# yakir1991/LoRa-SDR-Lightweight-Standalone-Library-

Hardware: AMD Instinct MI355X
Metric: Msymbols/s dechirp+FFT+argmax @ SF7 & SF12, 1/2/4/8 GPU; % HBM roofline (higher is better)
Workload: dtype f32; 1 GPU; SF7 BW125 osr1 LEGACY lora_demodulate + fused dechirp, 15625 frames x (2 sync + 64 data) symbols per GPU, noiseless; launch=eager, streams=3, sf=7, osr=1, frames_per_gpu=15625, data_symbols_per_frame=64, parallelism=frames sharded x1, no collective (gloo timing only), symbols_ok=True

## Files before the change

### lora-sdr-lightweight-standalone-library-_amd/csrc/lora_demod_fast.hip

```cpp
#include "../../include/lora_mi355x.h"
#include "lora_internal.h"

#include <algorithm>
#include <cstdlib>
#include <type_traits>
#include <utility>

#pragma clang fp contract(off)

namespace lora {
namespace {


template <int SF>
struct Geo {
  static constexpr int N = 1 << SF;
  static constexpr bool SMALL = SF <= 5;
  static constexpr int P = SMALL ? N : 16;
  static constexpr int T = N / P;
  static constexpr int R1 = SMALL ? N : ((SF & 1) ? 8 : 16);
  static constexpr int LOGR1 = SMALL ? SF : ((SF & 1) ? 3 : 4);
  static constexpr int G1 = P / R1;
  static constexpr bool R2FIRST = (SF & 1) != 0;
  static constexpr int X = N / R1;
// ... 676 lines not shown
      const auto xb = __builtin_amdgcn_permlane16_swap(best, best, false, false);
      const auto xs = __builtin_amdgcn_permlane16_swap(sec, sec, false, false);
      const auto xp = __builtin_amdgcn_permlane16_swap(pm, pm, false, false);
      best = xb[0], sec = xs[0], pm = xp[0];
      top2_merge(best, sec, pm, xb[1], xs[1], xp[1]);
    } else {
      static_assert(O == 32, "wave64");
      const auto xb = __builtin_amdgcn_permlane32_swap(best, best, false, false);
      const auto xs = __builtin_amdgcn_permlane32_swap(sec, sec, false, false);
      const auto xp = __builtin_amdgcn_permlane32_swap(pm, pm, false, false);
      best = xb[0], sec = xs[0], pm = xp[0];
      top2_merge(best, sec, pm, xb[1], xs[1], xp[1]);
    }
    spec_reduce_step<2 * O, W>(best, sec, pm);
  }
}
template <int SF>
__device__ __forceinline__ void spec_reduce(uint32_t& best, uint32_t& sec, float& pmf, int tid, uint32_t* scratch) {
  constexpr int T = Geo<SF>::T;
  uint32_t pm = __float_as_uint(pmf);
  spec_reduce_step<1, (T < 64 ? T : 64)>(best, sec, pm);
  if constexpr (T > 64) {
    const int w = tid >> 6;
    if ((tid & 63) == 0) {
      scratch[3 * w] = best;
      scratch[3 * w + 1] = sec;
      scratch[3 * w + 2] = pm;
    }
    __syncthreads();
    constexpr int WPS = T / 64;
    const int wb = (w / WPS) * WPS;
    best = scratch[3 * wb];
    sec = scratch[3 * wb + 1];
    pm = scratch[3 * wb + 2];
#pragma unroll
    for (int q = 1; q < WPS; ++q)
      top2_merge(best, sec, pm, scratch[3 * (wb + q)], scratch[3 * (wb + q) + 1], scratch[3 * (wb + q) + 2]);
  }
  pmf = __uint_as_float(pm);
}

template <int SF>
constexpr int demod_waves_per_eu() {
  return SF >= 6 ? 4 : 1;
}

template <int SF, bool SPEC>
constexpr int demod_twl_entries() {
  if constexpr (!SPEC || SF < 6) {
    return 0;
  } else {
    using G = Geo<SF>;
    return (G::RA == 16 ? 15 : 3) * G::MA_A;
  }
}


template <int SF>
constexpr size_t spec_dtl_offset() {
  return (((size_t)Geo<SF>::SPW * lds_row<SF>() + demod_twl_entries<SF, true>()) * sizeof(cf) + 15) & ~(size_t)15;
}
template <int SF>
constexpr bool spec_dtab() {
  return Geo<SF>::WAVE_LOCAL && Geo<SF>::NPASS == 2 &&
         4 * (spec_dtl_offset<SF>() + 2 * sizeof(cf) * Geo<SF>::N) <= 160 * 1024;
}
template <int SF>
constexpr size_t spec_lds_bytes() {
  constexpr bool pf2 = Geo<SF>::WAVE_LOCAL && Geo<SF>::NPASS == 2;
  return pf2 ? spec_dtl_offset<SF>() + (spec_dtab<SF>() ? 2 * sizeof(cf) * Geo<SF>::N : 16 * 8 * Geo<SF>::T)
             : sizeof(cf) * ((size_t)Geo<SF>::SPW * lds_row<SF>() + demod_twl_entries<SF, true>());
}

#define LORA_SPEC_BLOCKS(SPB, dblocks, frames, sync) ((dblocks) + ((sync) ? (2 * (frames) + (SPB) - 1) / (SPB) : 0))
template <int SF>
struct SpecGrid {
  static constexpr int SPB = Geo<SF>::WAVE_LOCAL ? 64 / Geo<SF>::T : Geo<SF>::SPW;
  static constexpr int BPG = Geo<SF>::WAVE_LOCAL ? 4 : 1;
  __host__ __device__ static constexpr int bpf(int per) { return (per + SPB - 1) / SPB; }
  static constexpr int64_t groups(int64_t frames, int per, bool sync) {
    return (LORA_SPEC_BLOCKS(SPB, frames * bpf(per), frames, sync) + BPG - 1) / BPG;
  }
};

__device__ __forceinline__ __amdgpu_buffer_rsrc_t raw_rsrc(const void* p) {
  return __builtin_amdgcn_make_buffer_rsrc(const_cast<void*>(p), (short)0, 0x7fffffff, 0x00020000);
}

struct SpecBlk {
  int64_t f, base;
  int s, jl, d, cg;
  bool valid, mis, nbr;
  float rate;
  int toff;
};
template <int SF, int SPM, int DW, bool RECIP>
__device__ __forceinline__ void spec_decode(const KArgs& a, int64_t bb, int bpf, int per, int gi, int l, bool fdiv,
                                            uint64_t mq, SpecBlk& B) {
  constexpr int SPB = SpecGrid<SF>::SPB, S0 = SPM == 2 ? 0 : 2;
  const __attribute__((address_space(4))) FrameParams* fps =
      (const __attribute__((address_space(4))) FrameParams*)a.fp_spec;
  if constexpr (RECIP)
    B.f = fdiv ? (bpf == 1 ? bb : (int64_t)(((uint64_t)(uint32_t)bb * mq) >> 32)) : bb / bpf;
  else
    B.f = bb / bpf;
  B.jl = (int)(bb - B.f * bpf) * SPB + gi;
  B.valid = B.jl < per;
  B.s = S0 + (B.valid ? B.jl : per - 1);
  B.rate = SPM == 2 ? 0.0f : fps[B.f].rate;
  B.toff = SPM == 2 ? 0 : fps[B.f].t_off;
  sym_base(B.s, Geo<SF>::N, a.frame_len, B.toff, B.base, B.cg);
  if constexpr (SPM == 1) B.cg = 0;
  B.d = (int)(B.base & (DW - 1));
  B.mis = __builtin_amdgcn_readfirstlane(__ballot(Geo<SF>::NPASS == 3 ? l < B.d : B.d != 0) != 0);
  B.nbr = false;
}
template <int SF>
__device__ __forceinline__ bool spec_next_is_neighbour(const KArgs& a, const SpecBlk& B, int per, int gi) {
  int64_t bnext;
  int cgn;
  sym_base(B.s + 1, Geo<SF>::N, a.frame_len, B.toff, bnext, cgn);
  return gi < SpecGrid<SF>::SPB - 1 && B.jl + 1 < per && bnext == B.base + Geo<SF>::N;
}

template <int SF, bool DTAB, bool DTL>
__device__ __forceinline__ float4 spec_table_pair(int pp, __amdgpu_buffer_rsrc_t rd, int vt, bool cg0, const cf* dq,
                                                  const float4* dl) {
  constexpr int N = Geo<SF>::N, T = Geo<SF>::T;
  if constexpr (DTAB) {
    const cf d0 = dq[2 * pp * T], d1 = dq[(2 * pp + 1) * T];
    return float4{d0.re, d0.im, d1.re, d1.im};
  } else if constexpr (DTL) {
    return cg0 ? dl[pp * T]
               : __builtin_bit_cast(float4, __builtin_amdgcn_raw_buffer_load_b128(rd, vt, pp * (N + T) * 16, 0));
  } else {
    return __builtin_bit_cast(float4, __builtin_amdgcn_raw_buffer_load_b128(rd, vt, pp * (N + T) * 16, 0));
  }
}
template <int SF, bool DTAB, bool DTL, int NP>
__device__ __forceinline__ void spec_table(const KArgs& a, int cg, int lr, const cf* dtab, const float4* dtl,
                                           float4 (&dt)[NP]) {
  const __amdgpu_buffer_rsrc_t rd = raw_rsrc(a.downP);
  const int vt = (cg + lr) * 16;
  bool cg0 = false;
  if constexpr (DTL && !DTAB) cg0 = __builtin_amdgcn_readfirstlane(__ballot(cg != 0) == 0);
#pragma unroll
  for (int pp = 0; pp < NP; ++pp) dt[pp] = spec_table_pair<SF, DTAB, DTL>(pp, rd, vt, cg0, dtab + cg + lr, dtl + lr);
}
template <int MODE, bool MAX, int P>
__device__ __forceinline__ float spec_dechirp_max(const v2f (&ld)[P + 1], const float4* dt, cf (&in)[P]) {
#pragma unroll
  for (int q = 0; q < P; ++q) in[q] = cf{ld[q].x, ld[q].y};
  if constexpr (MODE == 0) {
#pragma unroll
    for (int pp = 0; pp < P / 2; ++pp) {
      in[2 * pp] = pk_cmul_ref(in[2 * pp], cf{dt[pp].x, dt[pp].y});
      in[2 * pp + 1] = pk_cmul_ref(in[2 * pp + 1], cf{dt[pp].z, dt[pp].w});
    }
  }
  float pm = 0.0f;
  if constexpr (MAX) {
#pragma unroll
    for (int q = 0; q < P; ++q) pm = amax3(pm, in[q]);
  }
  return pm;
}
// ... 53 lines not shown
  const float scale = (legacy && p.scaled) ? p.scale : 1.0f;

  constexpr bool FMA = SPEC && FAST;
  constexpr int NTW = demod_twl_entries<SF, SPEC>();
  static_assert(NTW <= 256, "one staged twiddle per thread");
  cf* twl = rows + (size_t)SPW * rowc;
  cf tv{0.0f, 0.0f};
  if constexpr (NTW > 0) {
    if (tid < NTW) tv = a.twTA ? a.twTA[tid] : a.tw[twT_index(N, G::MA_A, tid / G::MA_A, tid % G::MA_A)];
  }
  cf in[P], z[P];
  if (SPEC && MODE == 0 && a.downP)
    gather_points<SF, true>(a, x, l, 1, N, cg, 1, true, 1.0f, in);
  else
    gather_points<SF>(a, x, l, osr, step, cg, legacy ? 1 : 2, dech, SPEC ? 1.0f : scale, in);
  if constexpr (NTW > 0) {
    if (tid < NTW) twl[tid] = tv;
    if constexpr (G::WAVE_LOCAL) __syncthreads();
  }
  float pm = 0.0f;
  if constexpr (SPEC) {
#pragma unroll
    for (int q = 0; q < P; ++q) pm = amax3(pm, in[q]);
  }
  rotate_place<SF, !RAW, FAST, FMA>(in, z, start, p.rate, hann, a.win, l);
  if constexpr (SPEC) asm volatile("" : "+v"(pm));
  float sec = 0.0f;
  const uint64_t lkey =
      fft_key<SF, false, FMA, (NTW > 0)>(z, rows + (size_t)g * rowc, l, a, SPEC ? &sec : nullptr, twl);
  const uint64_t key = symbol_key<SF>(lkey, tid, red);
  if (l == 0 && valid && a.syms) a.syms[f * a.sym_stride + (s - s0)] = (uint16_t)key_index(key);
  if constexpr (SPEC) {
    float r2 = lkey == key ? sec : key_value(lkey);
    group_reduce2<SF>(r2, pm, tid, reinterpret_cast<float*>(smem + 64));
    if (l == 0 && valid) {
      const int64_t per = a.total - s0;
      reinterpret_cast<float2*>(a.spec_marg)[f * per + (s - s0)] = make_float2(sqrtf(key_value(key)) - sqrtf(r2), pm);
    }
  }
}


template <int SF, int MODE, bool HANN = false, int OSRV = 1, int SPM = 0>
__global__ void __launch_bounds__(256) __attribute__((amdgpu_waves_per_eu(demod_waves_per_eu<SF>())))
k_spec_demod(KArgs a, int64_t frames, int rowc, int64_t gstride) {
  using G = Geo<SF>;
  constexpr int N = G::N, T = G::T, P = G::P, SPW = G::SPW;
  constexpr bool WL = G::WAVE_LOCAL;
  using SG = SpecGrid<SF>;
  constexpr int SPB = SG::SPB;
  constexpr int BPG = SG::BPG;
  constexpr int NTW = demod_twl_entries<SF, true>();
  constexpr bool OSRN = OSRV != 1;
  constexpr bool FOLD = SF <= 8 && !HANN;
  static_assert(P == 16 && (MODE == 0 || MODE == 1), "SF >= 6, LEGACY (osr 1, or OSRN)");
  static_assert(OSRV == 0 || OSRV == 1 || OSRV == 2 || OSRV == 4, "osr 1, 2, 4 or run time");
  static_assert(NTW <= 256, "one staged twiddle per thread");
  extern __shared__ __attribute__((aligned(16))) unsigned char smem[];
  __shared__ uint32_t red3[3 * 4];
  cf* rows = reinterpret_cast<cf*>(smem);
  cf* twl = rows + (size_t)SPW * rowc;
  const int tot = a.total;
  constexpr bool API = SPM == 1, RAWM = SPM == 2;
  constexpr int S0 = RAWM ? 0 : 2;
  const int per = tot - S0;
  constexpr bool DTL = WL && G::NPASS == 2 && !OSRN && MODE == 0;
  constexpr bool DTAB = DTL && spec_dtab<SF>();
  float4* dtl = reinterpret_cast<float4*>(smem + spec_dtl_offset<SF>());
  cf* dtab = reinterpret_cast<cf*>(smem + spec_dtl_offset<SF>());
  if (SPM != 0 && blockIdx.x == 0 && threadIdx.x < kFixStripes) a.fix_count[16 * threadIdx.x] = 0;
  if constexpr (NTW > 0) {
    const int tid = threadIdx.x;
    if (tid < NTW) twl[tid] = a.twTA ? a.twTA[tid] : a.tw[twT_index(N, G::MA_A, tid / G::MA_A, tid % G::MA_A)];
    if constexpr (DTAB) {
      for (int i = tid; i < 2 * N; i += 256) dtab[i] = a.down[i];
    } else if constexpr (DTL) {
      static_assert(8 * T <= 256, "one staged pair per thread");
      if (tid < 8 * T) dtl[tid] = reinterpret_cast<const float4*>(a.downP)[(tid / T) * (N + T) + tid % T];
    }
    __syncthreads();
  }
  const int bpf = SG::bpf(per);
  const int64_t dblocks = frames * bpf;
  const int64_t blocks = LORA_SPEC_BLOCKS(SPB, dblocks, frames, SPM == 0);
  const int64_t groups = (blocks + BPG - 1) / BPG;
  const int wave = __builtin_amdgcn_readfirstlane((int)(threadIdx.x >> 6));

  auto run_block = [&](auto sync_c, int64_t b, int64_t fb, int rb) {
    constexpr bool SYNC = decltype(sync_c)::value;
    int tid = threadIdx.x;
    asm volatile("" : "+v"(tid));
    const int g = SPW == 1 ? 0 : tid / T;
    const int l = tid % T;
    const int gi = WL ? (g % SPB) : g;
    int64_t f, fu;
    int s;
    bool valid;
    int rel = 0;
    if constexpr (!SYNC) {
      f = fu = fb;
      const int jl = rb * SPB + gi;
      valid = jl < per;
      s = S0 + (valid ? jl : per - 1);
    } else {
      const int64_t k0 = (b - dblocks) * SPB;
      int64_t k = k0 + gi;
      valid = k < 2 * frames;
      if (!valid) k = 2 * frames - 1;
      f = k >> 1;
      s = (int)(k & 1);
      fu = k0 >> 1;
      rel = (int)((f - fu) * a.frame_stride * 8);
    }
    const FrameParams fp = RAWM ? FrameParams{} : a.fp_spec[f];
    const float rate = RAWM ? 0.0f : fp.rate;
    const int toff = RAWM ? 0 : fp.t_off;
    const int step = OSRN ? a.step : N;
    int64_t base;
    int cg;
    sym_base(s, step, a.frame_len, toff, base, cg);
    if constexpr (API) cg = 0;
    cf in[P];
    float pm = 0.0f;
    int lr = l;
    if constexpr (OSRN) {
      const int osr = OSRV ? OSRV : a.osr;
      const __amdgpu_buffer_rsrc_t rx = raw_rsrc(a.iq + fu * a.frame_stride);
      const __amdgpu_buffer_rsrc_t rd = raw_rsrc(a.down);
      const int vo = rel + (int)(base + (int64_t)l * osr) * 8;
      const int vt = (cg + l * osr) * 8;
      const int so = T * osr * 8;
      if constexpr (OSRV == 4) {
        const bool odd = (l & 1) != 0;
        lr = odd ? T / 2 + (l >> 1) : (l >> 1);
        const int vo2 = rel + (int)base * 8 + 16 * l;
        const int vt2 = (cg + 2 * l) * 8;
#pragma unroll
        for (int q = 0; q < P; ++q) {
          cf e0;
#pragma unroll
          for (int h = 0; h < 2; ++h) {
            const int i = 2 * q + h;
            const float4 y2 = __builtin_bit_cast(float4, __builtin_amdgcn_raw_buffer_load_b128(rx, vo2, i * 2 * T * 8, 2 ));
            cf y0 = cf{y2.x, y2.y}, y1 = cf{y2.z, y2.w};
            if constexpr (MODE == 0) {
              const float4 d2 = __builtin_bit_cast(float4, __builtin_amdgcn_raw_buffer_load_b128(rd, vt2, i * 2 * T * 8, 0));
              y0 = pk_cmul_ref(y0, cf{d2.x, d2.y});
              y1 = pk_cmul_ref(y1, cf{d2.z, d2.w});
            }
            if constexpr (!SYNC) pm = amax3(amax3(pm, y0), y1);
            if (h == 0) {
              e0 = y0;
            } else {
              const cf m = cf{__int_as_float(__builtin_amdgcn_update_dpp(0, __float_as_int(y0.re), 0x111, 0xF, 0xF, false)),
                              __int_as_float(__builtin_amdgcn_update_dpp(0, __float_as_int(y0.im), 0x111, 0xF, 0xF, false))};
              in[q] = odd ? m : e0;
            }
          }
        }
      } else if constexpr (OSRV == 2) {
#pragma unroll
        for (int q = 0; q < P; ++q) {
          const float4 y2 = __builtin_bit_cast(float4, __builtin_amdgcn_raw_buffer_load_b128(rx, vo, q * so, 2 ));
          cf y0 = cf{y2.x, y2.y}, y1 = cf{y2.z, y2.w};
          if constexpr (MODE == 0) {
            const float4 d2 = __builtin_bit_cast(float4, __builtin_amdgcn_raw_buffer_load_b128(rd, vt, q * so, 0));
            y0 = pk_cmul_ref(y0, cf{d2.x, d2.y});
            y1 = pk_cmul_ref(y1, cf{d2.z, d2.w});
          }
          if constexpr (!SYNC) pm = amax3(amax3(pm, y0), y1);
          in[q] = y0;
        }
      } else {
#pragma unroll
      for (int q = 0; q < P; ++q) {
        for (int k = 0; k < osr; ++k) {
          cf y = __builtin_bit_cast(cf, __builtin_amdgcn_raw_buffer_load_b64(rx, vo + 8 * k, q * so, 2 ));
          if constexpr (MODE == 0)
            y = pk_cmul_ref(y, __builtin_bit_cast(cf, __builtin_amdgcn_raw_buffer_load_b64(rd, vt + 8 * k, q * so, 0)));
          if constexpr (!SYNC) pm = amax3(pm, y);
          if (k == 0) in[q] = y;
        }
      }
      }
    } else {
    constexpr int D = T < 8 ? T : 8;
    const int d = (int)(base & (D - 1));
    lr = (l - d) & (T - 1);
    v2f ld[P + 1];
    const __amdgpu_buffer_rsrc_t rx = raw_rsrc(a.iq + fu * a.frame_stride);
    const int vo = rel + (int)(base - d + l) * 8;
    float4 dt[MODE == 0 ? P / 2 : 1];
    const __amdgpu_buffer_rsrc_t rd = raw_rsrc(a.downP);
    const int vt = (cg + lr) * 16;
    constexpr int AUX = SYNC ? 0 : 2;
#pragma unroll
    for (int pp = 0; pp < P / 2; ++pp) {
      if constexpr (MODE == 0) dt[pp] = spec_table_pair<SF, false, false>(pp, rd, vt, false, nullptr, nullptr);
#pragma unroll
      for (int q = 2 * pp; q < 2 * pp + 2; ++q)
        ld[q] = __builtin_bit_cast(v2f, __builtin_amdgcn_raw_buffer_load_b64(rx, vo, q * T * 8, AUX));
    }
    if (__builtin_amdgcn_readfirstlane(__ballot(l < d) != 0)) {
      const bool late = l < d;
      ld[P] = __builtin_bit_cast(
          v2f, __builtin_amdgcn_raw_buffer_load_b64(rx, late ? vo : vo - T * 8, P * T * 8, AUX));
#pragma unroll
      for (int q = 0; q < P; ++q) ld[q] = late ? ld[q + 1] : ld[q];
    }
    pm = spec_dechirp_max<MODE, !SYNC>(ld, dt, in);
    }
    cf z[P], wz[P];
    {
      v2f F[P];
      spec_factors<SF>(rate, lr, F);
      spec_rotate_place<SF, HANN, FOLD>(in, z, F, a.win, lr, wz);
    }
    asm volatile("" : "+v"(pm));
    const uint64_t lk = fft_key<SF, false, true, (NTW > 0), true, false, NoHook, FOLD>(
        z, rows + (size_t)g * rowc, lr, a, nullptr, twl, nullptr, NoHook{}, nullptr, wz);
    const uint32_t lbest = (uint32_t)lk;
    uint32_t best = lbest, sec = (uint32_t)(lk >> 32);
    spec_reduce<SF>(best, sec, pm, tid, red3);
    if (valid) {
      constexpr int NG = (G::NPASS == 2 ? P / G::RA : P / G::RB);
      constexpr int ML = G::NPASS == 2 ? G::MA_A : G::MA_B;
      const int o = (int)(best & 15u);
      const uint32_t idx = (uint32_t)(lr + T * (o % NG) + ML * (o / NG));
      const float margin = spec_margin(best, sec);
      uint2* mg = reinterpret_cast<uint2*>(a.spec_marg) + f * tot + s;
      if constexpr (!SYNC) {
        if (lbest == best && a.syms) a.syms[f * a.sym_stride + (s - S0)] = (uint16_t)idx;
        if (l == 0) *mg = make_uint2(__float_as_uint(margin), __float_as_uint(pm));
      } else {
        if (lbest == best) *mg = make_uint2(__float_as_uint(margin), idx);
      }
    }
    block_sync<WL>();
  };
  int64_t grp0 = blockIdx.x;
  constexpr bool PL = SF == 7 && !HANN && WL && G::NPASS == 2 && !OSRN;
  const int64_t bstep = gstride * BPG;
  if constexpr (PL) {
    static_assert(T == 8 && P == 16 && G::G1 == 2 && G::R1 == 8 && G::LOGR1 == 3 && FOLD, "SF7 geometry");
    static_assert(MODE != 0 || (DTAB && NTW > 0), "the fused dechirp reads the staged doubled table");
    constexpr int DL = 16;
    const int tid0 = threadIdx.x;
    const int g = tid0 / T;
    const int l = tid0 % T;
    const int gi = g % SPB;
    float4 nx[P / 2 + 1];
    const bool fdiv = (uint64_t)dblocks * (uint64_t)bpf < (1ull << 32);
    const uint64_t mq = ((1ull << 32) + (uint64_t)bpf - 1) / (uint64_t)bpf;
    auto issue = [&](int64_t bb, SpecBlk& B) {
      spec_decode<SF, SPM, DL, true>(a, bb, bpf, per, gi, l, fdiv, mq, B);
      const __amdgpu_buffer_rsrc_t rx = raw_rsrc(a.iq + B.f * a.frame_stride);
      const int vo = (int)(B.base - B.d) * 8 + 16 * l;
#pragma unroll
      for (int j = 0; j < P / 2; ++j)
        nx[j] = __builtin_bit_cast(float4, __builtin_amdgcn_raw_buffer_load_b128(rx, vo, j * DL * 8, 2 ));
      if (B.mis) {
        B.nbr = spec_next_is_neighbour<SF>(a, B, per, gi);
        if (!B.nbr) {
          if (2 * l < B.d) {
            const v2f e0 = __builtin_bit_cast(v2f, __builtin_amdgcn_raw_buffer_load_b64(rx, vo, (P / 2) * DL * 8, 2));
            nx[P / 2].x = e0.x;
            nx[P / 2].y = e0.y;
          }
          if (2 * l + 1 < B.d) {
            const v2f e1 = __builtin_bit_cast(v2f, __builtin_amdgcn_raw_buffer_load_b64(rx, vo + 8, (P / 2) * DL * 8, 2));
            nx[P / 2].z = e1.x;
            nx[P / 2].w = e1.y;
          }
        }
      }
    };
    int64_t b = grp0 * BPG + wave;
    SpecBlk nb{};
    if (b < dblocks) issue(b, nb);
    for (; b < dblocks; b += bstep, grp0 += gstride) {
      const SpecBlk B = nb;
      float4(&ld)[P / 2 + 1] = nx;
      const int d = B.d;
      int r[2];
      bool late[2];
#pragma unroll
      for (int h = 0; h < 2; ++h) {
        const int x = 2 * l + h - d;
        late[h] = x < 0;
        r[h] = x & (DL - 1);
      }
      cf dv[MODE == 0 ? P : 1];
      if constexpr (MODE == 0) {
#pragma unroll
        for (int h = 0; h < 2; ++h) {
          const cf* dq = dtab + B.cg + r[h];
#pragma unroll
          for (int m = 0; m < P / 2; ++m) dv[h + 2 * m] = dq[DL * m];
        }
      }
      cf in[P];
      if (B.mis) {
        const int src = ((int)__lane_id() + T) & 63;
        const float4 n0 = {__shfl(ld[0].x, src, 64), __shfl(ld[0].y, src, 64), __shfl(ld[0].z, src, 64),
                           __shfl(ld[0].w, src, 64)};
        if (B.nbr) ld[P / 2] = n0;
#pragma unroll
        for (int m = 0; m < P / 2; ++m) {
          in[2 * m] = late[0] ? cf{ld[m + 1].x, ld[m + 1].y} : cf{ld[m].x, ld[m].y};
          in[2 * m + 1] = late[1] ? cf{ld[m + 1].z, ld[m + 1].w} : cf{ld[m].z, ld[m].w};
        }
      } else {
#pragma unroll
        for (int m = 0; m < P / 2; ++m) {
          in[2 * m] = cf{ld[m].x, ld[m].y};
          in[2 * m + 1] = cf{ld[m].z, ld[m].w};
        }
      }
      constexpr bool EARLY = MODE == 0;
      if constexpr (EARLY) {
        __builtin_amdgcn_sched_barrier(0);
        if (b + bstep < dblocks) issue(b + bstep, nb);
        __builtin_amdgcn_sched_barrier(0);
      }
      if constexpr (MODE == 0) {
#pragma unroll
        for (int q = 0; q < P; ++q) in[q] = pk_cmul_ref(in[q], dv[q]);
      }
// ... 45 lines not shown
      const int vo = (int)(B.base - B.d + l) * 8;
#pragma unroll
      for (int q = 0; q < P; ++q)
        nx[q] = __builtin_bit_cast(v2f, __builtin_amdgcn_raw_buffer_load_b64(rx, vo, q * T * 8, 2 ));
      if (B.mis) {
        if constexpr (P3) {
          nx[P] = __builtin_bit_cast(
              v2f, __builtin_amdgcn_raw_buffer_load_b64(rx, l < B.d ? vo : vo - T * 8, P * T * 8, 2 ));
        } else {
          B.nbr = spec_next_is_neighbour<SF>(a, B, per, gi);
          if (l < B.d && !B.nbr)
            nx[P] = __builtin_bit_cast(v2f, __builtin_amdgcn_raw_buffer_load_b64(rx, vo, P * T * 8, 2 ));
        }
      }
    };
    int64_t b = grp0 * BPG + (WL ? wave : 0);
    SpecBlk nb{};
    if (b < dblocks) issue(b, nb);
    for (; b < dblocks; b += bstep, grp0 += gstride) {
      const SpecBlk B = nb;
      v2f(&ld)[P + 1] = nx;
      const int d = B.d;
      const int lr = (l - d) & (T - 1);
      float4 dt[MODE == 0 ? P / 2 : 1];
      if constexpr (MODE == 0) spec_table<SF, DTAB, DTL>(a, B.cg, lr, dtab, dtl, dt);
      if (B.mis) {
        const bool late = l < d;
        if constexpr (!P3) {
          const int src = ((int)__lane_id() + T) & 63;
          const v2f n0 = {__shfl(ld[0].x, src, 64), __shfl(ld[0].y, src, 64)};
          if (late && B.nbr) ld[P] = n0;
        }
#pragma unroll
        for (int q = 0; q < P; ++q) ld[q] = late ? ld[q + 1] : ld[q];
      }
      cf in[P];
      float pm = spec_dechirp_max<MODE, true>(ld, dt, in);
      constexpr int NTB = G::RB == 16 ? 15 : 3;
      cf wb[P3 ? (P / G::RB) * NTB : 1];
      if constexpr (P3) {
#pragma unroll
        for (int gg = 0; gg < P / G::RB; ++gg) load_tw2<G::RB, G::MA_B>(wb + gg * NTB, (lr + T * gg) % G::MA_B, a.twTB2);
      }
      asm volatile("" : "+v"(pm));
      cf z[P], wz[P];
      {
        v2f F[P];
        spec_factors<SF>(B.rate, lr, F);
        spec_rotate_place<SF, HANN, FOLD>(in, z, F, a.win, lr, wz);
      }
      asm volatile("" : "+v"(pm));
      auto prefetch = [&]() {
        if (b + bstep < dblocks) issue(b + bstep, nb);
      };
      int cpre[G::G1];
      uint64_t lk;
      if constexpr (P3) {
#pragma unroll
        for (int h = 0; h < G::G1; ++h) cpre[h] = d == 0 ? cown[h] : (int)(a.rev[lr + T * h] >> G::LOGR1);
        lk = fft_key<SF, false, true, (NTW > 0), true, true, decltype(prefetch), FOLD>(
            z, rows + (size_t)g * rowc, lr, a, nullptr, twl, cpre, prefetch, wb, wz);
      } else {
        __builtin_amdgcn_sched_barrier(0);
        prefetch();
        __builtin_amdgcn_sched_barrier(0);
#pragma unroll
        for (int h = 0; h < G::G1; ++h) cpre[h] = __shfl(cown[h], lane0 + lr, 64);
        lk = fft_key<SF, false, true, (NTW > 0), true, true, NoHook, FOLD>(
            z, rows + (size_t)g * rowc, lr, a, nullptr, twl, cpre, NoHook{}, nullptr, wz);
      }
      const uint32_t lbest = (uint32_t)lk;
      uint32_t best = lbest, sec = (uint32_t)(lk >> 32);
      spec_reduce<SF>(best, sec, pm, tid0, red3);
      if (B.valid) spec_store_symbol<SF, S0>(a, B.f, B.s, l, lr, lbest, best, sec, pm);
      block_sync<WL>();
    }
  }
  for (int64_t grp = grp0; grp < groups; grp += gstride) {
    const int64_t b = grp * BPG + (WL ? wave : 0);
    if (WL && b >= blocks) break;
    if (b < dblocks) {
      const int64_t fb = b / bpf;
      run_block(std::false_type{}, b, fb, (int)(b - fb * bpf));
    } else {
      run_block(std::true_type{}, b, 0, 0);
    }
  }
}

template <int SF>
struct EstGeo {
  static constexpr int T = Geo<SF>::T;
  static constexpr int BLOCK = T >= 64 ? 256 : 64;
  static constexpr int SPB = BLOCK / T;
  static constexpr bool PAIR = SF >= 7 && Geo<SF>::WAVE_LOCAL && Geo<SF>::NPASS == 2;
};

template <int SF, int MODE>
__device__ __forceinline__ uint32_t exact_symbol(const KArgs& a, const cf* __restrict__ x,
                                                           const FrameParams& q, int s, cf* row, int l, int tid,
                                                           uint64_t* red) {
  using G = Geo<SF>;
  constexpr int N = G::N, P = G::P;
  constexpr bool DYN = MODE == 2;
  const int step = DYN ? a.step : N;
  const int osr = DYN ? a.osr : 1;
  const bool legacy = DYN ? a.mode != LORA_MODE_API : true;
  const bool dech = DYN ? (legacy && a.dechirp) : (MODE == 0);
  const bool hann = a.hann != 0;
  int64_t base;
  int cg;
  sym_base(s, step, a.frame_len, q.t_off, base, cg);
  const float start = q.rate * ((float)((uint32_t)s * (uint32_t)N) + (float)q.t_off / (float)osr);
  cf in[P], z[P];
  gather_points<SF>(a, x + base, l, osr, step, cg, legacy ? 1 : 2, dech, (legacy && q.scaled) ? q.scale : 1.0f, in);
  rotate_place<SF, true>(in, z, start, q.rate, hann, a.win, l);
  uint64_t key = fft_key<SF, false>(z, row, l, a);
  key = symbol_key<SF>(key, tid, red);
  block_sync<G::WAVE_LOCAL>();
  return key_index(key);
}

constexpr double kHwSinCosErr = 2.0e-7;

template <int SF, int LANES>
__device__ __forceinline__ void certify_list(const KArgs& a, int64_t f, const FrameParams& q, bool valid, int li) {
  constexpr int N = 1 << SF;
  const FrameParams qs = a.fp_spec[f];
  const int per = a.total - 2;
  const bool same_t = qs.t_off == q.t_off;
  constexpr int T = N >= 16 ? N / 16 : 1;
  const double u = 1.0 / 16777216.0;
  const double E = (8.0 * SF + 42.0) * u;
  const double drate = fabs((double)q.rate - (double)qs.rate);
  const double rmax = fmax(fabs((double)q.rate), fabs((double)qs.rate));
  const double tabs = (double)abs(q.t_off);
  const double e_spec = 36.0 * u * rmax * T + 16.0 * (1.87e-7 + 1.4143 * kHwSinCosErr) + 2.6e-6 + 9.6e-7;
  auto certified = [&](double d, double wmax, int s) {
    const double n1 = 2.0 * N * wmax;
    const double L = (double)(s + 1) * N + tabs;
    const double e_ref = u * rmax * (L + 2.0 * N);
    const double B = n1 * (drate * N + e_ref + e_spec + 2.0 * E);
    return same_t && d > 4.0 * B + 0x1p-60;
  };
  const uint2* __restrict__ mg = reinterpret_cast<const uint2*>(a.spec_marg) + f * a.total;
  bool sync_rej = false;
  if (a.mode != LORA_MODE_API) {
    const uint2 e = mg[li < 2 ? li : 0];
    const bool ok = certified((double)__uint_as_float(e.x), (double)__uint_as_float(a.maxbits[f]), li & 1);
    const uint32_t ok1 = (uint32_t)__shfl_down((int)ok, 1, 64), i1 = (uint32_t)__shfl_down((int)e.y, 1, 64);
    if (li == 0 && valid) {
      if (ok && ok1) {
        if (a.sync) {
          const unsigned shift = a.sf > 4 ? a.sf - 4 : 0;
          a.sync[f] = (uint8_t)((((e.y >> shift) & 0x0f) << 4) | ((i1 >> shift) & 0x0f));
        }
      } else {
        sync_rej = true;
      }
    }
  }
  if (valid) {
    uint64_t rejbits = 0;
#pragma unroll 8
    for (int j = li, k = 0; j < per; j += LANES, ++k) {
      const uint2 v = mg[2 + j];
      if (!certified((double)__uint_as_float(v.x), (double)__uint_as_float(v.y), 2 + j)) rejbits |= 1ull << k;
// ... 352 lines not shown

template <int SF, int MODE>
__global__ void __launch_bounds__(256) __attribute__((amdgpu_waves_per_eu(2)))
k_spec_fix(KArgs a, int rowc, int64_t grid) {
  using G = Geo<SF>;
  constexpr int T = G::T, SPW = G::SPW;
  extern __shared__ __attribute__((aligned(16))) unsigned char smem[];
  __shared__ uint64_t red[4];
  const int tid = threadIdx.x;
  const int g = SPW == 1 ? 0 : tid / T;
  const int l = tid % T;
  int64_t count = 0;
  unsigned cnt[kFixStripes];
#pragma unroll
  for (int t = 0; t < kFixStripes; ++t) {
    cnt[t] = __builtin_nontemporal_load(a.fix_count + 16 * t);
    count += cnt[t];
  }
  if (blockIdx.x == 0 && tid == 0 && count > 0) atomicAdd(a.spec_fix, (unsigned)count);
  cf* row = reinterpret_cast<cf*>(smem) + (size_t)g * rowc;
  for (int64_t r0 = 0; (int64_t)blockIdx.x + grid * r0 < count; r0 += SPW) {
    const int64_t i = (int64_t)blockIdx.x + grid * (r0 + g);
    const bool valid = i < count;
    int64_t k = valid ? i : count - 1;
    int t = 0;
#pragma unroll
    for (int u = 0; u < kFixStripes - 1; ++u)
      if (t == u && k >= (int64_t)cnt[u]) {
        k -= cnt[u];
        ++t;
      }
    const uint32_t* list = a.fix_list + 2 * (size_t)t * (size_t)a.fix_cap;
    const int64_t f = list[2 * k];
    const uint32_t j = list[2 * k + 1];
    const bool sync = j == 0xFFFFFFFFu;
    const FrameParams q = a.fp[f];
    const cf* __restrict__ x = a.iq + f * a.frame_stride;
    int lo = l;
    asm volatile("" : "+v"(lo));
    const int js = (a.mode == LORA_MODE_RAW ? 0 : 2) + (int)j;
    const uint32_t i0 = exact_symbol<SF, MODE>(a, x, q, sync ? 0 : js, row, lo, tid, red);
    const bool any_sync = G::WAVE_LOCAL ? __any(sync) : __syncthreads_or(sync);
    uint32_t i1 = 0;
    if (any_sync) i1 = exact_symbol<SF, MODE>(a, x, q, sync ? 1 : js, row, lo, tid, red);
    if (l == 0 && valid) {
      if (!sync) {
        if (a.syms) a.syms[f * a.sym_stride + j] = (uint16_t)i0;
      } else if (a.sync) {
        const unsigned shift = a.sf > 4 ? a.sf - 4 : 0;
        a.sync[f] = (uint8_t)((((i0 >> shift) & 0x0f) << 4) | ((i1 >> shift) & 0x0f));
      }
    }
  }
}

template <int SF>
int row_complex() {
  return lds_row<SF>();
}

template <int SF, int MODE>
__global__ void __launch_bounds__(64) __attribute__((amdgpu_waves_per_eu(4)))
k_est_split(KArgs a, int64_t frames, int rowc) {
  using G = Geo<SF>;
  constexpr int N = G::N, T = G::T, P = G::P;
  constexpr int FPW = 64 / (2 * T);
  static_assert(2 * T <= 64 && P == 16, "SF 6-9");
  constexpr bool dech = MODE == 0;
  extern __shared__ __attribute__((aligned(16))) unsigned char smem[];
  __shared__ FrameParams sp[FPW];
  __shared__ float tail[FPW][2][4];
  const int tid = threadIdx.x;
  if (blockIdx.x == 0 && tid < kFixStripes) a.fix_count[16 * tid] = 0;
  const int g2 = tid / T;
  const int fg = g2 >> 1;
  const int sym = g2 & 1;
  const int l = tid % T;
  const int l2 = tid % (2 * T);
  const int64_t f0 = (int64_t)blockIdx.x * FPW + fg;
  const bool valid = f0 < frames;
  const int64_t f = valid ? f0 : frames - 1;
  const cf* __restrict__ x = a.iq + f * a.frame_stride;
  cf* row = reinterpret_cast<cf*>(smem) + (size_t)g2 * rowc;
  auto frame_max = [&](float v) {
#pragma unroll
    for (int o = T; o > 0; o >>= 1) v = fmaxf(v, __shfl_xor(v, o, 64));
    return v;
  };
  FrameParams q;
  {
    cf in[P], z[P];
    gather_points<SF>(a, x + (int64_t)sym * N, l, 1, N, 0, 1, dech, 1.0f, in);
    float mo = 0.0f;
#pragma unroll
    for (int k = 0; k < P; ++k) mo = amax3(mo, in[k]);
    asm volatile("" : "+v"(mo));
    const float m01 = frame_max(mo);
    const int scaled = m01 > 1.0f;
    const float scale = scaled ? 1.0f / m01 : 1.0f;
    if (scaled) {
#pragma unroll
      for (int k = 0; k < P; ++k) in[k] = cscale(in[k], scale);
    }
    rotate_place<SF, false>(in, z, 0.0f, 0.0f, a.hann != 0, a.win, l);
    uint64_t key = fft_key<SF, true>(z, row, l, a);
    key = group_max(key, T);
    if (l == 0) {
      const uint32_t idx = key_index(key);
      const uint32_t im1 = idx > 0 ? idx - 1 : N - 1, ip1 = idx < (uint32_t)N - 1 ? idx + 1 : 0;
      const cf L = row[lds_slot<SF>((int)im1)], R = row[lds_slot<SF>((int)ip1)], B = row[lds_slot<SF>((int)idx)];
      const float fi = detect_findex(key_value(key), L, R);
      const bool take = key_value(key) > 0.0f;
      tail[fg][sym][0] = take ? (float)idx : 0.0f;
      tail[fg][sym][1] = take ? fi : 0.0f;
      tail[fg][sym][2] = lm_atan2f(take ? B.im : 0.0f, take ? B.re : 0.0f);
    }
    wave_sync();
    if (l2 == 0) {
      float sum_index = 0.0f, phase_diff = 0.0f;
      sum_index += tail[fg][0][0] + tail[fg][0][1];
      sum_index += tail[fg][1][0] + tail[fg][1][1];
      float d = tail[fg][1][2] - tail[fg][0][2];
      while (d > PI_F) d -= 2.0f * PI_F;
      while (d < -PI_F) d += 2.0f * PI_F;
      phase_diff += d;
      const float avg_index = sum_index / 2.0f;
      const float cfo_coarse = avg_index / (float)N;
      const float cfo_fine = (phase_diff / 1.0f) / (2.0f * PI_F * (float)N);
      const float cfo = cfo_coarse + cfo_fine;
      const float frac = avg_index - floorf(avg_index + 0.5f);
      const float avg_t = (float)0u / 2.0f;
      const float toff = avg_t - frac * (float)N * 1.0f;
      FrameParams qe;
      qe.cfo = cfo;
      qe.toff = toff;
      qe.t_off = (int)roundf(toff);
      qe.rate = -2.0f * PI_F * cfo / (float)N;
      qe.scale = scale;
      qe.scaled = scaled;
      qe.pad0 = qe.pad1 = 0;
      sp[fg] = qe;
      if (valid) a.fp_spec[f] = qe;
    }
    wave_sync();
    q = sp[fg];
    {
      int64_t b2, bl;
      int cg;
      sym_base(2, N, a.frame_len, q.t_off, b2, cg);
      sym_base(a.total - 1, N, a.frame_len, q.t_off, bl, cg);
      const int64_t xend = bl + N;
      float m = mo;
      for (int64_t j = 2 * (int64_t)N + l2; j < b2; j += 2 * T) {
        cf v = x[j];
        if (dech) v = cmul(v, a.down[j % N]);
        m = fmaxf(m, fmaxf(fabsf(v.re), fabsf(v.im)));
      }
      for (int64_t j = xend + l2; j < a.frame_len; j += 2 * T) {
        cf v = x[j];
        if (dech) v = cmul(v, a.down[j % N]);
        m = fmaxf(m, fmaxf(fabsf(v.re), fabsf(v.im)));
      }
      m = frame_max(m);
      if (l2 == 0 && valid) a.spec_max[f] = __float_as_uint(m);
    }
  }
}

template <int SF, int MODE>
__global__ void __launch_bounds__(64) __attribute__((amdgpu_waves_per_eu(4)))
k_cert_split(KArgs a, int64_t frames, int rowc) {
  using G = Geo<SF>;
  constexpr int N = G::N, T = G::T, P = G::P;
  constexpr int FPW = 64 / (2 * T);
  static_assert(2 * T <= 64 && P == 16, "SF 6-9");
  constexpr bool dech = MODE == 0;
  extern __shared__ __attribute__((aligned(16))) unsigned char smem[];
  __shared__ FrameParams sp[FPW];
  __shared__ float tail[FPW][2][4];
  const int tid = threadIdx.x;
  const int g2 = tid / T;
  const int fg = g2 >> 1;
  const int sym = g2 & 1;
  const int l = tid % T;
  const int l2 = tid % (2 * T);
  const int64_t f0 = (int64_t)blockIdx.x * FPW + fg;
  const bool valid = f0 < frames;
  const int64_t f = valid ? f0 : frames - 1;
  const cf* __restrict__ x = a.iq + f * a.frame_stride;
  cf* row = reinterpret_cast<cf*>(smem) + (size_t)g2 * rowc;
  const int per = a.total - 2;
  const FrameParams qg = load_fp(a.fp_spec + f);
  float maxv = l2 == 0 ? __uint_as_float(a.maxbits[f]) : 0.0f;
  {
    const float2* __restrict__ mg = reinterpret_cast<const float2*>(a.spec_marg) + f * a.total + 2;
#pragma unroll 4
    for (int j = l2; j < per; j += 2 * T) maxv = fmaxf(maxv, mg[j].y);
#pragma unroll
    for (int o = T; o > 0; o >>= 1) maxv = fmaxf(maxv, __shfl_xor(maxv, o, 64));
  }
  const int scaled = maxv > 1.0f;
  const float scale = scaled ? 1.0f / maxv : 1.0f;
  const bool guessed = scaled ? (qg.scaled != 0 && qg.scale == scale) : qg.scaled == 0;
  if (__builtin_amdgcn_readfirstlane(__ballot(!guessed) == 0)) {
    if (l2 == 0) {
      store_fp(sp + fg, qg);
      if (valid) {
        store_fp(a.fp + f, qg);
        if (a.cfo) a.cfo[f] = qg.cfo;
        if (a.toff) a.toff[f] = qg.toff;
        if (a.max_amp) a.max_amp[f] = maxv;
      }
    }
  } else {
    {
      cf in[P], z[P];
      gather_points<SF>(a, x + (int64_t)sym * N, l, 1, N, 0, 1, dech, 1.0f, in);
      if (scaled) {
#pragma unroll
        for (int q = 0; q < P; ++q) in[q] = cscale(in[q], scale);
      }
      rotate_place<SF, false>(in, z, 0.0f, 0.0f, a.hann != 0, a.win, l);
      uint64_t key = fft_key<SF, true>(z, row, l, a);
      key = group_max(key, T);
      if (l == 0) {
        const uint32_t idx = key_index(key);
        const uint32_t im1 = idx > 0 ? idx - 1 : N - 1, ip1 = idx < (uint32_t)N - 1 ? idx + 1 : 0;
        const cf L = row[lds_slot<SF>((int)im1)], R = row[lds_slot<SF>((int)ip1)], B = row[lds_slot<SF>((int)idx)];
        const float fi = detect_findex(key_value(key), L, R);
        const bool take = key_value(key) > 0.0f;
        tail[fg][sym][0] = take ? (float)idx : 0.0f;
        tail[fg][sym][1] = take ? fi : 0.0f;
        tail[fg][sym][2] = lm_atan2f(take ? B.im : 0.0f, take ? B.re : 0.0f);
      }
      wave_sync();
    }
    if (l2 == 0) {
      float sum_index = 0.0f, phase_diff = 0.0f;
      sum_index += tail[fg][0][0] + tail[fg][0][1];
      sum_index += tail[fg][1][0] + tail[fg][1][1];
      float d = tail[fg][1][2] - tail[fg][0][2];
      while (d > PI_F) d -= 2.0f * PI_F;
      while (d < -PI_F) d += 2.0f * PI_F;
      phase_diff += d;
      const float avg_index = sum_index / 2.0f;
      const float cfo_coarse = avg_index / (float)N;
      const float cfo_fine = (phase_diff / 1.0f) / (2.0f * PI_F * (float)N);
      const float cfo = cfo_coarse + cfo_fine;
      const float frac = avg_index - floorf(avg_index + 0.5f);
      const float avg_t = (float)0u / 2.0f;
      const float toff = avg_t - frac * (float)N * 1.0f;
      FrameParams qe;
      qe.cfo = cfo;
      qe.toff = toff;
      qe.t_off = (int)roundf(toff);
      qe.rate = -2.0f * PI_F * cfo / (float)N;
      qe.scale = scale;
      qe.scaled = scaled;
      qe.pad0 = qe.pad1 = 0;
      sp[fg] = qe;
      if (valid) {
        a.fp[f] = qe;
        if (a.cfo) a.cfo[f] = cfo;
        if (a.toff) a.toff[f] = toff;
        if (a.max_amp) a.max_amp[f] = maxv;
      }
    }
  }
  wave_sync();
  const FrameParams q = sp[fg];
  certify_list<SF, 2 * T>(a, f, q, valid, l2);
}

template <class... P, class... A>
bool launch_lds(void (*k)(P...), int64_t grid, int block, size_t lds, hipStream_t st, A&&... args) {
  if (lds > 160 * 1024) return false;
  if (lds > 64 * 1024 &&
      hipFuncSetAttribute((const void*)k, hipFuncAttributeMaxDynamicSharedMemorySize, (int)lds) != hipSuccess)
    return false;
  launch(k, dim3((unsigned)grid), dim3((unsigned)block), lds, st, std::forward<A>(args)...);
  return true;
}

template <int SF>
bool launch_split(void (*k)(KArgs, int64_t, int), const KArgs& a, int64_t frames, hipStream_t st) {
  constexpr int FPW = 64 / (2 * Geo<SF>::T);
  const int rowc = row_complex<SF>();
  return launch_lds(k, (frames + FPW - 1) / FPW, 64, sizeof(cf) * (size_t)(2 * FPW) * rowc, st, a, frames, rowc);
}

template <int SF, int MODE, int SPEC = 0>
bool launch_est_mode(const KArgs& a, int64_t frames, hipStream_t st) {
  using G = Geo<SF>;
  constexpr int T = G::T;
  constexpr int BLOCK = T >= 64 ? 256 : 64;
  constexpr int SPB = BLOCK / T;
  const int rowc = row_complex<SF>();
  const size_t lds = G::NPASS == 1 ? 16 : sizeof(cf) * (size_t)SPB * rowc * (EstGeo<SF>::PAIR && MODE <= 1 ? 2 : 1);
  return launch_lds(k_est_fast<SF, MODE, SPEC>, (frames + SPB - 1) / SPB, BLOCK, lds, st, a, frames, rowc);
}

template <int SF>
bool launch_est_sf(const KArgs& a, int64_t frames, hipStream_t st) {
  const bool simple = a.mode == LORA_MODE_LEGACY && a.osr == 1 && !a.hann;
  if (simple && a.dechirp) return launch_est_mode<SF, 0>(a, frames, st);
  if (simple) return launch_est_mode<SF, 1>(a, frames, st);
  return launch_est_mode<SF, 2>(a, frames, st);
}

template <int SF, int MODE, bool FAST = false, bool SPEC = false>
bool launch_mode(const KArgs& a, int s0, int64_t work, hipStream_t st) {
  using G = Geo<SF>;
  const int rowc = row_complex<SF>();
  const size_t lds = G::NPASS == 1 ? 16 : sizeof(cf) * ((size_t)G::SPW * rowc + demod_twl_entries<SF, SPEC>());
  return launch_lds(k_demod_fast<SF, MODE, FAST, SPEC>, (work + G::SPW - 1) / G::SPW, 256, lds, st, a, s0, work, rowc);
}

constexpr int kSpecWgPerCu = 4;
int device_cus() {
  static int cache[64] = {};
  int dev = 0;
  if (hipGetDevice(&dev) != hipSuccess || dev < 0 || dev >= 64) return 256;
  if (!cache[dev]) {
    int n = 0;
    if (hipDeviceGetAttribute(&n, hipDeviceAttributeMultiprocessorCount, dev) != hipSuccess || n <= 0) n = 256;
    cache[dev] = n;
  }
  return cache[dev];
}

template <int SF, int MODE, bool HANN, int OSRV, int SPM = 0>
bool launch_spec_demod_w(const KArgs& a, int64_t frames, hipStream_t st) {
  using G = Geo<SF>;
  using SG = SpecGrid<SF>;
  const int per = a.total - (SPM == 2 ? 0 : 2);
  const int64_t groups = SG::groups(frames, per, SPM == 0);
  const bool persist = G::WAVE_LOCAL || (G::NPASS == 3 && a.osr == 1);
  const int64_t cap = persist ? (int64_t)device_cus() * kSpecWgPerCu : groups;
  const int64_t grid = groups < cap ? groups : cap;
  return launch_lds(k_spec_demod<SF, MODE, HANN, OSRV, SPM>, grid, 256, spec_lds_bytes<SF>(), st, a, frames,
                    row_complex<SF>(), grid);
}
template <int SF, int MODE>
bool launch_spec_demod(const KArgs& a, int64_t frames, hipStream_t st) {
  if (a.osr > 1) {
    if (a.hann) return launch_spec_demod_w<SF, MODE, true, 0>(a, frames, st);
    if (a.osr == 2) return launch_spec_demod_w<SF, MODE, false, 2>(a, frames, st);
    if (a.osr == 4) return launch_spec_demod_w<SF, MODE, false, 4>(a, frames, st);
    return launch_spec_demod_w<SF, MODE, false, 0>(a, frames, st);
  }
  return a.hann ? launch_spec_demod_w<SF, MODE, true, 1>(a, frames, st)
                : launch_spec_demod_w<SF, MODE, false, 1>(a, frames, st);
}

template <int SF, int MODE>
bool launch_spec_fix(const KArgs& a, int64_t frames, hipStream_t st) {
  using G = Geo<SF>;
  const int rowc = row_complex<SF>();
  const size_t lds = sizeof(cf) * (size_t)G::SPW * rowc;
  const int64_t most = (frames * (int64_t)(a.total - 1) + G::SPW - 1) / G::SPW;
  const int64_t cap = (int64_t)device_cus();
  const int64_t grid = std::max<int64_t>(1, std::min(most, cap));
  return launch_lds(k_spec_fix<SF, MODE>, grid, 256, lds, st, a, rowc, grid);
}

template <int SF>
bool launch_spec_sf(const KArgs& a, int64_t frames, int stage, hipStream_t st) {
  if constexpr (SF < 6) {
    return false;
  } else {
    if (a.mode == LORA_MODE_RAW) {
      if constexpr (SF > 9) {
        return false;
      } else {
        if (stage == 1) {
          if (a.hann)
            return a.dechirp ? launch_spec_demod_w<SF, 0, true, 1, 2>(a, frames, st)
                             : launch_spec_demod_w<SF, 1, true, 1, 2>(a, frames, st);
          return a.dechirp ? launch_spec_demod_w<SF, 0, false, 1, 2>(a, frames, st)
                           : launch_spec_demod_w<SF, 1, false, 1, 2>(a, frames, st);
        }
        if (stage == 2) {
          const int64_t n = frames * (int64_t)a.total;
          launch(k_cert_raw<SF>, dim3((unsigned)((n + 255) / 256)), dim3(256), 0, st, a, frames);
          return true;
        }
        if (stage == 3) return launch_spec_fix<SF, 2>(a, frames, st);
        return false;
      }
    }
    if (a.mode == LORA_MODE_API) {
      if (stage == 0) return launch_est_mode<SF, 2, 0>(a, frames, st);
      if (stage == 1)
        return a.hann ? launch_spec_demod_w<SF, 0, true, 1, 1>(a, frames, st)
                      : launch_spec_demod_w<SF, 0, false, 1, 1>(a, frames, st);
      if (stage == 2) return launch_est_mode<SF, 2, 2>(a, frames, st);
      return launch_spec_fix<SF, 2>(a, frames, st);
    }
    if (a.osr > 1) {
      if (stage == 0) return launch_est_mode<SF, 2, 1>(a, frames, st);
      if (stage == 1)
        return a.dechirp ? launch_spec_demod<SF, 0>(a, frames, st) : launch_spec_demod<SF, 1>(a, frames, st);
      if (stage == 2) return launch_est_mode<SF, 2, 2>(a, frames, st);
      return launch_spec_fix<SF, 2>(a, frames, st);
    }
    if constexpr (SF <= 9) {
      if (stage == 0) return launch_split<SF>(a.dechirp ? k_est_split<SF, 0> : k_est_split<SF, 1>, a, frames, st);
      if (stage == 2) return launch_split<SF>(a.dechirp ? k_cert_split<SF, 0> : k_cert_split<SF, 1>, a, frames, st);
    }
    if (stage == 3) return a.dechirp ? launch_spec_fix<SF, 0>(a, frames, st) : launch_spec_fix<SF, 1>(a, frames, st);
    if (stage == 0) return a.dechirp ? launch_est_mode<SF, 0, 1>(a, frames, st) : launch_est_mode<SF, 1, 1>(a, frames, st);
    if (stage == 1)
      return a.dechirp ? launch_spec_demod<SF, 0>(a, frames, st) : launch_spec_demod<SF, 1>(a, frames, st);
    return a.dechirp ? launch_est_mode<SF, 0, 2>(a, frames, st) : launch_est_mode<SF, 1, 2>(a, frames, st);
  }
}

template <int SF>
bool launch_sf(const KArgs& a, int s0, int64_t work, hipStream_t st) {
  const bool simple = a.mode == LORA_MODE_LEGACY && a.osr == 1 && !a.hann;
  if (a.mode == LORA_MODE_RAW) return launch_mode<SF, 3>(a, s0, work, st);
  if (a.fast_rot) {
    if (simple && a.dechirp) return launch_mode<SF, 0, true>(a, s0, work, st);
    if (simple) return launch_mode<SF, 1, true>(a, s0, work, st);
    return launch_mode<SF, 2, true>(a, s0, work, st);
  }
  if (simple && a.dechirp) return launch_mode<SF, 0>(a, s0, work, st);
  if (simple) return launch_mode<SF, 1>(a, s0, work, st);
  return launch_mode<SF, 2>(a, s0, work, st);
}

template <int LO, int HI, class F>
bool dispatch_sf(int sf, F&& f) {
  if constexpr (LO > HI)
    return false;
  else
    return sf == LO ? f(std::integral_constant<int, LO>{}) : dispatch_sf<LO + 1, HI>(sf, f);
}

}


bool launch_spec(const KArgs& a, int64_t frames, int stage, hipStream_t st) {
  return dispatch_sf<6, 12>(a.sf, [&](auto sf) { return launch_spec_sf<sf()>(a, frames, stage, st); });
}

bool launch_est_fast(const KArgs& a, int64_t frames, hipStream_t st) {
  if (a.total < 2 || a.est_only || a.mode == LORA_MODE_RAW) return false;
  return dispatch_sf<2, 12>(a.sf, [&](auto sf) { return launch_est_sf<sf()>(a, frames, st); });
}

bool launch_demod_fast(const KArgs& a, int s0, int64_t work, hipStream_t st) {
  return dispatch_sf<2, 12>(a.sf, [&](auto sf) { return launch_sf<sf()>(a, s0, work, st); });
}

}
```

Before: 5387 Msymbols/s.

## Fold sync-symbol spectral demod into the estimation split kernel for small SF

For SF<=9 at osr 1, the two sync-symbol spectral blocks no longer run inside the persistent spec-demod kernel. Each frame's sync FFT/argmax now runs at the end of the k_est_split kernel, which already holds the frame's samples and parameters, with twiddles staged into extra LDS. This removes the sync-block tail and its dispatch branch from the main spec kernel. In exchange the estimation kernel needs more LDS and registers, which may lower its occupancy.

```diff
diff --git a/lora-sdr-lightweight-standalone-library-_amd/csrc/lora_demod_fast.hip b/lora-sdr-lightweight-standalone-library-_amd/csrc/lora_demod_fast.hip
--- a/lora-sdr-lightweight-standalone-library-_amd/csrc/lora_demod_fast.hip
+++ b/lora-sdr-lightweight-standalone-library-_amd/csrc/lora_demod_fast.hip
@@ -782,6 +782,10 @@
     return (LORA_SPEC_BLOCKS(SPB, frames * bpf(per), frames, sync) + BPG - 1) / BPG;
   }
 };
+template <int SF, int OSRV, int SPM>
+constexpr bool spec_sync_blocks() {
+  return SPM == 0 && (SF > 9 || OSRV != 1);
+}
 
 __device__ __forceinline__ __amdgpu_buffer_rsrc_t raw_rsrc(const void* p) {
   return __builtin_amdgcn_make_buffer_rsrc(const_cast<void*>(p), (short)0, 0x7fffffff, 0x00020000);
@@ -1001,7 +1005,8 @@
   }
   const int bpf = SG::bpf(per);
   const int64_t dblocks = frames * bpf;
-  const int64_t blocks = LORA_SPEC_BLOCKS(SPB, dblocks, frames, SPM == 0);
+  constexpr bool SYNCB = spec_sync_blocks<SF, OSRV, SPM>();
+  const int64_t blocks = LORA_SPEC_BLOCKS(SPB, dblocks, frames, SYNCB);
   const int64_t groups = (blocks + BPG - 1) / BPG;
   const int wave = __builtin_amdgcn_readfirstlane((int)(threadIdx.x >> 6));
 
@@ -1162,7 +1167,7 @@
   const int64_t bstep = gstride * BPG;
   if constexpr (PL) {
     static_assert(T == 8 && P == 16 && G::G1 == 2 && G::R1 == 8 && G::LOGR1 == 3 && FOLD, "SF7 geometry");
-    static_assert(MODE != 0 || (DTAB && NTW > 0), "the fused dechirp reads the staged doubled table");
+    static_assert(NTW > 0 && (MODE != 0 || DTAB), "staged twiddles; the fused dechirp reads the staged doubled table");
     constexpr int DL = 16;
     const int tid0 = threadIdx.x;
     const int g = tid0 / T;
@@ -1374,7 +1379,7 @@
     if (b < dblocks) {
       const int64_t fb = b / bpf;
       run_block(std::false_type{}, b, fb, (int)(b - fb * bpf));
-    } else {
+    } else if constexpr (SYNCB) {
       run_block(std::true_type{}, b, 0, 0);
     }
   }
@@ -1893,6 +1898,8 @@
   const int64_t f = valid ? f0 : frames - 1;
   const cf* __restrict__ x = a.iq + f * a.frame_stride;
   cf* row = reinterpret_cast<cf*>(smem) + (size_t)g2 * rowc;
+  constexpr int NTW = demod_twl_entries<SF, true>();
+  cf* twl = reinterpret_cast<cf*>(smem) + (size_t)(2 * FPW) * rowc;
   auto frame_max = [&](float v) {
 #pragma unroll
     for (int o = T; o > 0; o >>= 1) v = fmaxf(v, __shfl_xor(v, o, 64));
@@ -1906,6 +1913,8 @@
 #pragma unroll
     for (int k = 0; k < P; ++k) mo = amax3(mo, in[k]);
     asm volatile("" : "+v"(mo));
+    for (int i = tid; i < NTW; i += 64)
+      twl[i] = a.twTA ? a.twTA[i] : a.tw[twT_index(N, G::MA_A, i / G::MA_A, i % G::MA_A)];
     const float m01 = frame_max(mo);
     const int scaled = m01 > 1.0f;
     const float scale = scaled ? 1.0f / m01 : 1.0f;
@@ -1976,6 +1985,51 @@
       if (l2 == 0 && valid) a.spec_max[f] = __float_as_uint(m);
     }
   }
+  auto sync_spec = [&](auto hann_c) {
+    constexpr bool HANN = decltype(hann_c)::value;
+    constexpr bool FOLD = SF <= 8 && !HANN;
+    int64_t base;
+    int cg;
+    sym_base(sym, N, a.frame_len, q.t_off, base, cg);
+    const cf* __restrict__ xw = x + base + l;
+    cf in[P];
+#pragma unroll
+    for (int k = 0; k < P; ++k) in[k] = xw[T * k];
+    if constexpr (dech) {
+      const __amdgpu_buffer_rsrc_t rd = raw_rsrc(a.downP);
+      const int vt = (cg + l) * 16;
+#pragma unroll
+      for (int pp = 0; pp < P / 2; ++pp) {
+        const float4 dt = spec_table_pair<SF, false, false>(pp, rd, vt, false, nullptr, nullptr);
+        in[2 * pp] = pk_cmul_ref(in[2 * pp], cf{dt.x, dt.y});
+        in[2 * pp + 1] = pk_cmul_ref(in[2 * pp + 1], cf{dt.z, dt.w});
+      }
+    }
+    cf z[P], wz[P];
+    {
+      v2f F[P];
+      spec_factors<SF>(q.rate, l, F);
+      spec_rotate_place<SF, HANN, FOLD>(in, z, F, a.win, l, wz);
+    }
+    const uint64_t lk = fft_key<SF, false, true, true, true, false, NoHook, FOLD>(z, row, l, a, nullptr, twl, nullptr,
+                                                                                NoHook{}, nullptr, wz);
+    const uint32_t lbest = (uint32_t)lk;
+    uint32_t best = lbest, sec = (uint32_t)(lk >> 32);
+    float pm = 0.0f;
+    spec_reduce<SF>(best, sec, pm, tid, nullptr);
+    if (valid && lbest == best) {
+      constexpr int NG = G::NPASS == 2 ? P / G::RA : P / G::RB;
+      constexpr int ML = G::NPASS == 2 ? G::MA_A : G::MA_B;
+      const int o = (int)(best & 15u);
+      const uint32_t idx = (uint32_t)(l + T * (o % NG) + ML * (o / NG));
+      reinterpret_cast<uint2*>(a.spec_marg)[f * a.total + sym] =
+          make_uint2(__float_as_uint(spec_margin(best, sec)), idx);
+    }
+  };
+  if (a.hann)
+    sync_spec(std::true_type{});
+  else
+    sync_spec(std::false_type{});
 }
 
 template <int SF, int MODE>
@@ -2094,10 +2148,11 @@
 }
 
 template <int SF>
-bool launch_split(void (*k)(KArgs, int64_t, int), const KArgs& a, int64_t frames, hipStream_t st) {
+bool launch_split(void (*k)(KArgs, int64_t, int), const KArgs& a, int64_t frames, hipStream_t st, int extra = 0) {
   constexpr int FPW = 64 / (2 * Geo<SF>::T);
   const int rowc = row_complex<SF>();
-  return launch_lds(k, (frames + FPW - 1) / FPW, 64, sizeof(cf) * (size_t)(2 * FPW) * rowc, st, a, frames, rowc);
+  return launch_lds(k, (frames + FPW - 1) / FPW, 64, sizeof(cf) * ((size_t)(2 * FPW) * rowc + extra), st, a, frames,
+                    rowc);
 }
 
 template <int SF, int MODE, int SPEC = 0>
@@ -2145,7 +2200,7 @@
   using G = Geo<SF>;
   using SG = SpecGrid<SF>;
   const int per = a.total - (SPM == 2 ? 0 : 2);
-  const int64_t groups = SG::groups(frames, per, SPM == 0);
+  const int64_t groups = SG::groups(frames, per, spec_sync_blocks<SF, OSRV, SPM>());
   const bool persist = G::WAVE_LOCAL || (G::NPASS == 3 && a.osr == 1);
   const int64_t cap = persist ? (int64_t)device_cus() * kSpecWgPerCu : groups;
   const int64_t grid = groups < cap ? groups : cap;
@@ -2216,7 +2271,9 @@
       return launch_spec_fix<SF, 2>(a, frames, st);
     }
     if constexpr (SF <= 9) {
-      if (stage == 0) return launch_split<SF>(a.dechirp ? k_est_split<SF, 0> : k_est_split<SF, 1>, a, frames, st);
+      if (stage == 0)
+        return launch_split<SF>(a.dechirp ? k_est_split<SF, 0> : k_est_split<SF, 1>, a, frames, st,
+                                demod_twl_entries<SF, true>());
       if (stage == 2) return launch_split<SF>(a.dechirp ? k_cert_split<SF, 0> : k_cert_split<SF, 1>, a, frames, st);
     }
     if (stage == 3) return a.dechirp ? launch_spec_fix<SF, 0>(a, frames, st) : launch_spec_fix<SF, 1>(a, frames, st);
```

New measurement: 5374 Msymbols/s. No clear change (-0.2%).
